# alanqrwang/keymorph

Hardware: AMD Instinct MI355X
Metric: volume-pairs/sec (fwd+bwd) at 256^3, 512 kp, TPS (higher is better)
Workload: dtype f32

## Files before the change

include/keymorph_hip.h:

```cpp
#ifndef KEYMORPH_HIP_H
#define KEYMORPH_HIP_H
#include <stddef.h>
#include <stdint.h>
#ifdef __cplusplus
extern "C" {
#endif

#define KMH_EINVAL (-22)
#define KMH_ABI_VERSION 1
int kmh_abi_version(void);

int kmh_grid_sample3d_fwd(const float* x, const float* grid, float* out, int N, int C, int D, int H,
                          int W, int Do, int Ho, int Wo, int mode, void* stream);
int kmh_grid_sample3d_bwd_grid(const float* x, const float* grid, const float* gout, float* dgrid,
                               int N, int C, int D, int H, int W, int Do, int Ho, int Wo, void* stream);
int kmh_grid_sample3d_bwd_input(const float* grid, const float* gout, float* dx, int N, int C, int D,
                                int H, int W, int Do, int Ho, int Wo, void* stream);

size_t kmh_reduce_ws_bytes(void);
int kmh_mse_fwd(const float* a, const float* b, long long n, float* out, void* ws, void* stream);
int kmh_mse_bwd(const float* a, const float* b, const float* gscale, long long n, float* da, void* stream);
int kmh_warp_mse_fwd(const float* x, const float* grid, const float* fixed, float* out, float* out_loss,
                     int N, int C, int D, int H, int W, int Do, int Ho, int Wo, void* ws, void* stream);
int kmh_warp_mse_fwd_grad(const float* x, const float* grid, const float* fixed, float* out, float* out_loss,
// ... 102 lines not shown
size_t kmh_conv3d_pack_bf_bytes(int Cout, int Cin, int transposed, int terms);
int kmh_conv3d_pack_weight_bf(const float* w, void* packed, int Cout, int Cin, int transposed, int terms,
                              const float* wscale, void* stream);
size_t kmh_conv3d_fwd_bf_stats_ws_bytes(int N, int D, int H, int W, int Cout, int rows_per_wave);
int kmh_conv3d_fwd_bf(const float* x, const float* scale, const float* shift, const float* mask, const void* packed,
                      const float* bias, float* y, int N, int D, int H, int W, int Cin, int Cout, int relu_in,
                      int relu_out, int terms, int rows_per_wave, const float* ascale, const float* wscale,
                      void* stats_ws, double* stats_out, int in_blocked, const float* addend, void* stream);
int kmh_conv3d_fwd_bf_set_dispatch(int mode);
int kmh_conv3d_fwd_bf_split_ok(int N, int D, int H, int W, int Cin, int Cout, int terms);
int kmh_conv3d_fwd_bf_sparse_ok(int N, int D, int H, int W, int Cin, int Cout, int terms);
int kmh_conv3d_fwd_bf_sparse(const float* xp, const unsigned char* winners, const void* packed, const float* bias, float* y,
                             int N, int D, int H, int W, int Cin, int Cout, int relu_out, int terms, const float* ascale,
                             const float* wscale, void* stats_ws, double* stats_out, void* stream);
int kmh_conv3d_fwd_bf_variant(int N, int D, int H, int W, int Cin, int Cout, int terms, int has_mask, int has_addend);
int kmh_conv3d_fwd_bf_pool_ok(int N, int D, int H, int W, int Cin, int Cout, int terms);
int kmh_conv3d_fwd_bf_pool(const float* x, const float* scale, const float* shift, const void* packed, float* yp,
                           unsigned char* arg, int N, int D, int H, int W, int Cin, int Cout, int relu_in, int terms,
                           const float* ascale, const float* wscale, void* stats_ws, double* stats_out, int in_blocked,
                           void* stream);
size_t kmh_conv3d_up2_pack_bytes(int Cout, int Cl, int terms);
int kmh_conv3d_up2_pack_weight(const float* w, void* packed, int Cout, int Ctot, int cofs, int Cl, int terms,
                               const float* wscale, void* stream);
size_t kmh_conv3d_up2_dgrad_pack_bytes(int Cout, int Cl, int terms);
int kmh_conv3d_up2_dgrad_pack_weight(const float* w, void* packed, int Cout, int Ctot, int cofs, int Cl, int terms,
                                     const float* wscale, void* stream);
size_t kmh_conv3d_up2_dgrad_stats_ws_bytes(int N, int Dl, int Hl, int Wl, int Cl);
int kmh_conv3d_up2_dgrad(const float* dz, const void* packed, float* ds, int N, int Dl, int Hl, int Wl, int Cl, int Cout,
                         int terms, const float* dscale, const float* wscale, void* stats_ws, double* stats_out,
                         int in_blocked ,
// ... 158 lines not shown
```

keymorph_amd/_lib.py:

```python
from __future__ import annotations

import ctypes as C
import os

from .build import LIBPATH

_f = C.c_void_p
_i = C.c_int
_ll = C.c_longlong
_sz = C.c_size_t

PROTOS = {
    "kmh_abi_version": (_i, []),
    "kmh_grid_sample3d_fwd": (_i, [_f, _f, _f, _i, _i, _i, _i, _i, _i, _i, _i, _i, _f]),
    "kmh_grid_sample3d_bwd_grid": (_i, [_f, _f, _f, _f, _i, _i, _i, _i, _i, _i, _i, _i, _f]),
    "kmh_grid_sample3d_bwd_input": (_i, [_f, _f, _f, _i, _i, _i, _i, _i, _i, _i, _i, _f]),
    "kmh_reduce_ws_bytes": (_sz, []),
    "kmh_mse_fwd": (_i, [_f, _f, _ll, _f, _f, _f]),
    "kmh_mse_bwd": (_i, [_f, _f, _f, _ll, _f, _f]),
    "kmh_warp_mse_fwd": (_i, [_f, _f, _f, _f, _f, _i, _i, _i, _i, _i, _i, _i, _i, _f, _f]),
    "kmh_warp_mse_fwd_grad": (_i, [_f, _f, _f, _f, _f, _f, _i, _i, _i, _i, _i, _i, _i, _i, _f, _f]),
    "kmh_scale_unless_one": (_i, [_f, _ll, _f, _f]),
    "kmh_dice_sums": (_i, [_f, _f, _i, _ll, _f, _f, _f]),
    "kmh_rows_axpby": (_i, [_f, _f, _f, _f, _i, _ll, _f, _f]),
# ... 40 lines not shown
    "kmh_mi_hist_ranges": (_i, [_f, _f, _f, _i, _ll, _i, _f, _f]),
    "kmh_warp_mi_ws_bytes": (_sz, [_i, _i, _i, _i, _i]),
    "kmh_warp_mi_hist": (_i, [_f, _f, _f, _f, _i, _i, _i, _i, _i, _f, _f]),
    "kmh_warp_mi_bwd": (_i, [_f, _f, _f, _f, _f, _f, _i, _i, _i, _i, _i, _f, _f, _f]),
    "kmh_affine_build_matrix": (_i, [_f, _f, _f, _f, _f, _i, _f]),
    "kmh_affine_points_bwd": (_i, [_f, _f, _f, _f, _f, _i, _i, _f]),
    "kmh_com3d_fwd": (_i, [_f, _f, _f, _i, _i, _i, _i, _i, _f, _f]),
    "kmh_com3d_bwd": (_i, [_f, _f, _f, _f, _i, _i, _i, _i, _i, _f]),
    "kmh_conv3d_pack_weight": (_i, [_f, _f, _i, _i, _i, _f]),
    "kmh_conv3d_fwd": (_i, [_f, _f, _f, _f, _f, _f, _f, _i, _i, _i, _i, _i, _i, _i, _i, _f]),
    "kmh_conv3d_pack_bf_bytes": (_sz, [_i, _i, _i, _i]),
    "kmh_conv3d_pack_weight_bf": (_i, [_f, _f, _i, _i, _i, _i, _f, _f]),
    "kmh_conv3d_fwd_bf": (_i, [_f, _f, _f, _f, _f, _f, _f, _i, _i, _i, _i, _i, _i, _i, _i, _i, _i, _f, _f, _f, _f, _i, _f, _f]),
    "kmh_conv3d_fwd_bf_set_dispatch": (_i, [_i]),
    "kmh_conv3d_fwd_bf_variant": (_i, [_i, _i, _i, _i, _i, _i, _i, _i, _i]),
    "kmh_conv3d_fwd_bf_pool_ok": (_i, [_i, _i, _i, _i, _i, _i, _i]),
    "kmh_conv3d_fwd_bf_split_ok": (_i, [_i, _i, _i, _i, _i, _i, _i]),
    "kmh_conv3d_fwd_bf_sparse_ok": (_i, [_i, _i, _i, _i, _i, _i, _i]),
    "kmh_conv3d_fwd_bf_sparse": (_i, [_f, _f, _f, _f, _f, _i, _i, _i, _i, _i, _i, _i, _i, _f, _f, _f, _f, _f]),
    "kmh_conv3d_fwd_bf_pool": (_i, [_f, _f, _f, _f, _f, _f, _i, _i, _i, _i, _i, _i, _i, _i, _f, _f, _f, _f, _i, _f]),
    "kmh_conv3d_up2_dgrad_pack_bytes": (_sz, [_i, _i, _i]),
    "kmh_conv3d_up2_dgrad_pack_weight": (_i, [_f, _f, _i, _i, _i, _i, _i, _f, _f]),
    "kmh_conv3d_up2_dgrad_stats_ws_bytes": (_sz, [_i, _i, _i, _i, _i]),
    "kmh_conv3d_up2_dgrad": (_i, [_f, _f, _f, _i, _i, _i, _i, _i, _i, _i, _f, _f, _f, _f, _i, _f]),
    "kmh_up2_boxsum": (_i, [_f, _f, _i, _i, _i, _i, _i, _i, _f]),
    "kmh_up2_wgrad_gemm_ws_bytes": (_sz, [_i, _i, _i, _i]),
    "kmh_up2_wgrad_gemm": (_i, [_f, _f, _f, _i, _i, _i, _i, _i, _f, _f, _f, _f, _f, _f]),
    "kmh_up2_wgrad_fold_ok": (_i, [_i, _i, _i]),
    "kmh_up2_wgrad_fold_ws_bytes": (_sz, [_i, _i, _i, _i, _i, _i]),
    "kmh_up2_wgrad_fold": (_i, [_f, _f, _f, _i, _i, _i, _i, _i, _i, _i, _f, _f, _f, _f, _i, _f, _f]),
# ... 178 lines not shown
```

keymorph_amd/csrc/conv_bf.hip:

```cpp
#include <atomic>
#include <cstdio>
#include <cstdlib>
#include "conv_split.h"
#include "stats_final.h"
#include <type_traits>

namespace {

constexpr int TX = 32, TZ = 2;
constexpr int HX = TX + 2, HZ = TZ + 2;
constexpr int NSTEP = 14;
constexpr int BF_TPB = 256;

constexpr int NSTEP_Z = 18;
template <int TERMS>
__global__ __launch_bounds__(256) void pack_weight_bf_kernel(const float* __restrict__ w, __bf16* __restrict__ out,
                                                             int Cout, int Cin, int CoutP, int nchunk,
                                                             int transposed, int zpair,
                                                             const float* __restrict__ wscale ) {
  const int Co = transposed ? Cin : Cout, Ci = transposed ? Cout : Cin;
  const int nstep = zpair ? NSTEP_Z : NSTEP;
  const long long total = (long long)nchunk * nstep * 2 * CoutP * 8;
  for (long long e = (long long)blockIdx.x * 256 + threadIdx.x; e < total; e += (long long)gridDim.x * 256) {
    const int c = (int)(e & 7);
// ... 732 lines not shown
#define KMH_S_DEEP 1
#endif
#ifndef KMH_S_CW
#define KMH_S_CW 1
#endif
#ifndef KMH_S_STAMPALL
#define KMH_S_STAMPALL 0
#endif
#ifndef KMH_S_IL
#define KMH_S_IL 1
#endif
#ifndef KMH_S_DEEP_RING_V
#define KMH_S_DEEP_RING_V 0
#endif

template <int NT, bool ZP = false, bool SPLIT = false, bool POOL = false, bool AMP = false, bool SPARSE = false>
__global__ __launch_bounds__(S_TPB, 1) void conv3_fwd_s_kernel(
    const float* __restrict__ x, const float* __restrict__ scale, const float* __restrict__ shift,
    const bf16x8* __restrict__ wp, const float* __restrict__ bias, float* __restrict__ y, int D, int H, int W, int Cin,
    int Cout, int CoutP, int relu_in, int relu_out, int tiles_x, int tiles_y, int tiles_z, int tiles_zp,
    const float* __restrict__ ascale, const float* __restrict__ wscale, double* __restrict__ stats_partial,
    int in_blocked, const float* __restrict__ addend, int total_items, int N, long long* __restrict__ trace,
    unsigned* __restrict__ pool_arg = nullptr) {
  constexpr int TERMS = 2, MR = ZP ? 4 : S_MR, NST = ZP ? NSTEP_Z : NSTEP;
  static_assert(!ZP || NT == 1, "z-paired tiles are for Cout <= 16");
  static_assert(ZP == SPLIT, "the z-paired tile is launched on pre-split operands only (fp32 operands: conv3_fwd_g_kernel<1, true>)");
  static_assert(!POOL || (NT == 1 && !ZP), "the pooling epilogue is built for the 32-wide tile");
  static_assert(!SPARSE || (SPLIT && ZP && !AMP && TX % 2 == 0 && GTY % 2 == 0 && GTZ % 2 == 0), "pooled operand: the pre-split arm, even brick origins");
  extern __shared__ __attribute__((aligned(16))) unsigned char gsm[];
  int* sOff = reinterpret_cast<int*>(gsm + 2 * S_BUF_BYTES);
  float* sCoef = reinterpret_cast<float*>(gsm + 2 * S_BUF_BYTES + S_OFF_BYTES);
  const int tid = threadIdx.x, lane = tid & 63;
  const int wv = __builtin_amdgcn_readfirstlane(tid >> 6);
  const int li = lane & 31, lh = lane >> 5;
  const int ncog = ZP ? 1 : (Cout + 32 * NT - 1) / (32 * NT);
  const int tyz = (tiles_y + 7) >> 3;
  struct Item { int n, cog, bx, by, bz; };
  const int total_all = N * total_items;
  auto decode = [&](int vb, Item& it) -> bool {
    const int gitem = xcd_remap(vb, total_all);
    it.n = gitem / total_items;
    const int item = gitem - it.n * total_items;
    it.cog = item % ncog;
    const int brick = item / ncog;
    const int lz8 = brick & 7, ly8 = (brick >> 3) & 7, patch = brick >> 6;
    const int pyi = patch % tyz, rest = patch / tyz;
    const int pzi = rest % tiles_zp;
    it.bx = rest / tiles_zp; it.by = pyi * 8 + ly8; it.bz = pzi * 8 + lz8;
// ... 76 lines not shown
      const int v0_ = r * S_TPB + t_, v = v0_ < GPL ? v0_ : GPL - 1;
      const int lx = v % HX, ly = (v / HX) % GHY, lz = v / (HX * GHY);
      int gx = x0 + lx - 1, gy = y0 + ly - 1, gz = z0 + lz - 1;
      const bool in = (v0_ < GPL) && ((unsigned)gx < (unsigned)W) && ((unsigned)gy < (unsigned)H) && ((unsigned)gz < (unsigned)D);
      bits |= (in ? 1u : 0u) << r;
      gx = gx < 0 ? 0 : (gx > W - 1 ? W - 1 : gx);
      gy = gy < 0 ? 0 : (gy > H - 1 ? H - 1 : gy);
      gz = gz < 0 ? 0 : (gz > D - 1 ? D - 1 : gz);
      const int off = ((gz * H + gy) * W + gx) * (in_blocked ? KC : Cin);
      sOff[r * S_TPB + t_] = off;
      sOff[(8 + r) * S_TPB + t_] = off + 4;
    }
    return bits;
  };
  typedef float kmh_f4 __attribute__((ext_vector_type(4)));
  constexpr bool DEEP = (NT == 1) && !ZP && !SPLIT && (KMH_S_DEEP != 0);
  constexpr bool CW = !SPLIT && (KMH_S_CW != 0);
  constexpr int CD = DEEP ? 3 : (CW ? 2 : 1);
  constexpr int RQ = CD + 1;
  kmh_f4 rawq[RQ][2];
  auto raw_issue = [&](int n, int ch, int slot, int off0, int off1) {
    const float* base = sample_base(n) + ch * chunk_stride;
    const float* p0 = base + off0;
    const float* p1 = base + off1;
    if constexpr (CW) {
      asm volatile("global_load_dwordx4 %0, %1, off" : "=v"(rawq[slot][0]) : "v"(p0) : "memory");
      asm volatile("global_load_dwordx4 %0, %1, off" : "=v"(rawq[slot][1]) : "v"(p1) : "memory");
    } else {
      rawq[slot][0] = *reinterpret_cast<const kmh_f4*>(p0);
      rawq[slot][1] = *reinterpret_cast<const kmh_f4*>(p1);
    }
  };
// ... 12 lines not shown
      case 6: asm volatile("s_waitcnt vmcnt(6)" ::: "memory"); break;
      case 7: asm volatile("s_waitcnt vmcnt(7)" ::: "memory"); break;
      case 8: asm volatile("s_waitcnt vmcnt(8)" ::: "memory"); break;
      default: asm volatile("s_waitcnt vmcnt(0)" ::: "memory"); break;
    }
  };
  int coef_n = -1;
  auto fill_coef = [&](int n_) {
    for (int e = tid; e < Cin; e += S_TPB) {
      sCoef[e] = (scale ? scale[n_ * Cin + e] : 1.f) * sA;
      sCoef[S_COEF + e] = (scale ? shift[n_ * Cin + e] : 0.f) * sA;
    }
    coef_n = n_;
  };
  const float relu_floor = relu_in ? 0.f : -__builtin_inff();
  auto convert1 = [&](int ch, unsigned bits, int pb, int i, const kmh_f4 r0, const kmh_f4 r1) {
    const float4 a0 = *reinterpret_cast<const float4*>(sCoef + ch * KC), a1 = *reinterpret_cast<const float4*>(sCoef + ch * KC + 4);
    const float4 b0 = *reinterpret_cast<const float4*>(sCoef + S_COEF + ch * KC), b1 = *reinterpret_cast<const float4*>(sCoef + S_COEF + ch * KC + 4);
    const float csc[8] = {a0.x, a0.y, a0.z, a0.w, a1.x, a1.y, a1.z, a1.w};
    const float csh[8] = {b0.x, b0.y, b0.z, b0.w, b1.x, b1.y, b1.z, b1.w};
    bf16x8* B8 = reinterpret_cast<bf16x8*>(gsm + pb * S_BUF_BYTES);
    const int v = tid + i * S_TPB;
    const float raw[8] = {r0.x, r0.y, r0.z, r0.w, r1.x, r1.y, r1.z, r1.w};
    const bool in = (bits >> i) & 1u;
    const float lo = in ? relu_floor : 0.f, hi = in ? __builtin_inff() : 0.f;
    float val[8];
#pragma unroll
    for (int j = 0; j < 8; ++j) val[j] = __builtin_amdgcn_fmed3f(raw[j] * csc[j] + csh[j], lo, hi);
    bf16x8 parts[TERMS];
    split8<TERMS>(val, parts);
#pragma unroll
    for (int t = 0; t < TERMS; ++t) B8[t * S_PLANE + v] = parts[t];
  };

  auto dma_piece = [&](int n, int ch, int buf, int p, int off) {
    const float* src = sample_base(n) + ch * chunk_stride + off + 4 * (p & 1);
    unsigned char* dst = gsm + buf * S_BUF_BYTES + ((p & 1) * S_PLANE + (p >> 1) * S_TPB + wv * 64) * 16;
    __builtin_amdgcn_global_load_lds((kmh_glb_ptr)src, (kmh_lds_ptr)dst, 16, 0, 0);
  };
  typedef unsigned sp_u4 __attribute__((ext_vector_type(4)));
  const sp_u4* const spTab = reinterpret_cast<const sp_u4*>(sOff);
  kmh_f4 spg[2][2];
  typedef unsigned sp_u2 __attribute__((ext_vector_type(2)));
  sp_u2 spw[2];
  unsigned sph[4], spl[4], spP[4], spM[4], spB = 0;
  auto sp_issue = [&](int n, int ch) {
    const long long cells = vox >> 3;
// ... 115 lines not shown
    for (int t = s_ - BA + 1; t < s_; ++t) yb += NBL + nr(t);
    return yr < yb ? yr : yb;
  };
  auto a_offset = [&](int s) -> int {
    constexpr int last_tap = ZP ? 35 : 26;
    const int tapA = 2 * s, tapB = (2 * s + 1 > last_tap) ? last_tap : 2 * s + 1;
    const int offA = ((tapA / 9) * GHY + (tapA / 3) % 3) * HX + tapA % 3;
    const int offB = ((tapB / 9) * GHY + (tapB / 3) % 3) * HX + tapB % 3;
    return lh ? offB : offA;
  };

  int tr_n = 0;
  auto stamp = [&]() {
    if (trace && blockIdx.x == 0 && tid == 0 && tr_n < 240) trace[tr_n++] = __builtin_readcyclecounter();
  };
  unsigned cv_in = fill_offsets(cur);
  unsigned cv_brick_next = 0u;
  if constexpr (SPARSE) {
    sp_issue(cur.n, 0);
    asm volatile("s_waitcnt vmcnt(0)" ::: "memory");
    sp_tie();
#pragma unroll
    for (int c = 0; c < 2; ++c)
#pragma unroll
      for (int part = 0; part < SP_PARTS; ++part) sp_part(c, part, 0);
  } else if constexpr (SPLIT) {
#pragma unroll
    for (int p = 0; p < S_NLD; ++p) dma_piece(cur.n, 0, 0, p, sOff[(p >> 1) * S_TPB + tid]);
    asm volatile("s_waitcnt vmcnt(0)" ::: "memory");
  } else {
    fill_coef(cur.n);
    __syncthreads();
#pragma unroll
    for (int i = 0; i < S_NCV; ++i) {
      raw_issue(cur.n, 0, 0, sOff[i * S_TPB + tid], sOff[(8 + i) * S_TPB + tid]);
      asm volatile("s_waitcnt vmcnt(0)" ::: "memory");
      if (CW) raw_tie(0);
      convert1(0, cv_in, 0, i, rawq[0][0], rawq[0][1]);
    }
  }
  o0 = lh * CoutP + cur.cog * (32 * NT) + li;
#pragma unroll
  for (int d = 0; d < BA; ++d) b_issue(d);
  if (SPLIT || DEEP) asm volatile("s_waitcnt vmcnt(0)" ::: "memory");
  int pb = 0;
  for (;;) {
    const bool more = next_item(vb, nxt);
    const int co0 = cur.cog * (32 * NT);
    const int n = cur.n;
    const int boff = lh * CoutP + co0 + li;
    f32x16 acc[MR][NT];
#pragma unroll
    for (int m = 0; m < MR; ++m)
#pragma unroll
      for (int t = 0; t < NT; ++t)
#pragma unroll
        for (int r = 0; r < 16; ++r) acc[m][t][r] = 0.f;

    for (int ch = 0; ch < nchunk; ++ch) {
      stamp();
      asm volatile("s_waitcnt lgkmcnt(0)" ::: "memory");
      __builtin_amdgcn_s_barrier();
      stamp();
      const bf16x8* sIn = reinterpret_cast<const bf16x8*>(gsm + pb * S_BUF_BYTES);
      const bool last_ch = ch + 1 == nchunk;
      const int nn = (last_ch && more) ? nxt.n : n, nch = last_ch ? 0 : ch + 1;
      unsigned cv_next = last_ch ? 0u : cv_in;
      if (!SPLIT && nn != coef_n) {
        fill_coef(nn);
        __syncthreads();
      }
      const int co0n = ((last_ch && more) ? nxt.cog : cur.cog) * (32 * NT);
      int vr = vrow;
      asm volatile("" : "+v"(vr));
      int dof0 = 0, dof1 = 0;
      bf16x8 a[2][MR][TERMS];
      {
        const int ab = vr + a_offset(0);
#pragma unroll
        for (int m = 0; m < MR; ++m)
// ... 61 lines not shown
        } else {
        if (SPLIT || !(s >= 1 + CD && s < 9 + CD)) __builtin_amdgcn_sched_group_barrier(0x100, 64, 0);
        if (!SPLIT && s >= 1 + CD && s < 9 + CD) {
          __builtin_amdgcn_sched_group_barrier(0x100, 64, 0);
          __builtin_amdgcn_sched_group_barrier(0x008, 6, 0);
#pragma unroll
          for (int k = 0; k < NMF - 6; ++k) {
            __builtin_amdgcn_sched_group_barrier(0x002, 3, 0);
            __builtin_amdgcn_sched_group_barrier(0x008, 1, 0);
          }
        }
        }
        __builtin_amdgcn_sched_barrier(0);
        __builtin_amdgcn_sched_barrier(0);
        if (KMH_S_STAMPALL || s == 0 || s == 9 || s == NST - 1) stamp();
      }
      if (!last_ch) pb ^= 1;
    }

    if (SPLIT || DEEP) asm volatile("s_waitcnt vmcnt(0)" ::: "memory");
    const int x0 = cur.bx * TX, y0 = cur.by * GTY, z0 = cur.bz * GTZ;
    constexpr int CH = 32 * NT;
    constexpr int L4 = CH / 4;
    constexpr int VPI = 64 / L4;
    const long long sbrick = ((long long)n * tiles_z * tiles_y * tiles_x + ((long long)cur.bz * tiles_y + cur.by) * tiles_x + cur.bx);
    unsigned char* sEp = gsm + pb * S_BUF_BYTES;
    float* tile0 = reinterpret_cast<float*>(sEp) + wv * (2 * 32 * CH);
    const int c4 = lane % L4, vx = lane / L4;
    const int col = 4 * c4;
    const int pl = ZP ? col >> 4 : 0;
// ... 109 lines not shown
#pragma unroll
      for (int j = 0; j < 4; ++j) {
        d1[j] = (double)st1[j]; d2[j] = (double)st2[j];
#pragma unroll
        for (int o = L4; o < 64; o <<= 1) { d1[j] += __shfl_xor(d1[j], o); d2[j] += __shfl_xor(d2[j], o); }
      }
      if (POOL) stamp();
      __syncthreads();
      double* sred = reinterpret_cast<double*>(sEp);
      if (lane < L4) {
#pragma unroll
        for (int j = 0; j < 4; ++j) { sred[((wv * CH) + col + j) * 2] = d1[j]; sred[((wv * CH) + col + j) * 2 + 1] = d2[j]; }
      }
      __syncthreads();
      const int ncol = ZP ? 16 : CH;
      if (tid < 2 * ncol) {
        const int k = tid & 1, c = tid >> 1;
        const int cch = ZP ? c : co0 + c;
        if (cch < Cout) {
          double sum = 0.0;
#pragma unroll
          for (int w4 = 0; w4 < 4; ++w4) {
            sum += sred[(w4 * CH + c) * 2 + k];
            if (ZP) sum += sred[(w4 * CH + 16 + c) * 2 + k];
          }
          stats_partial[(sbrick * Cout + cch) * 2 + k] = sum;
        }
      }
    }
    stamp();
    if (!more) break;
    cur = nxt;
    cv_in = cv_brick_next;
    pb ^= 1;
  }
  asm volatile("s_waitcnt vmcnt(0)" ::: "memory");
}

}
static inline bool use_zpair(int Cout) { return Cout <= 16; }

KMH_API size_t kmh_conv3d_pack_bf_bytes(int Cout, int Cin, int transposed, int terms) {
  const int Co = transposed ? Cin : Cout, Ci = transposed ? Cout : Cin;
  return (size_t)((Ci + 7) / 8) * terms * (use_zpair(Co) ? NSTEP_Z : NSTEP) * 2 * cout_pad(Co) * 8 * sizeof(__bf16);
}

KMH_API int kmh_conv3d_pack_weight_bf(const float* w, void* packed, int Cout, int Cin, int transposed, int terms,
                                      const float* wscale, void* stream) {
  const int Co = transposed ? Cin : Cout, Ci = transposed ? Cout : Cin;
  const int nchunk = (Ci + 7) / 8, CoutP = cout_pad(Co), zp = use_zpair(Co);
  const long long total = (long long)nchunk * (zp ? NSTEP_Z : NSTEP) * 2 * CoutP * 8;
// ... 63 lines not shown
  if (int e = allow_lds(conv3_fwd_g_kernel<NT, ZP, POOL>, G_LDS_BYTES)) return e;
  const PersistentGrid g = persistent_grid(N, D, H, W, ZP ? 1 : ceil_div(Cout, 32 * NT));
  long long* trace = trace_begin(s);
  conv3_fwd_g_kernel<NT, ZP, POOL><<<dim3(g.wgs), G_TPB, G_LDS_BYTES, s>>>(x, scale, shift, wp, bias, y, D, H, W, Cin, Cout, CoutP,
                                                                           relu_in, relu_out, g.tx, g.ty, g.tz, g.tzp, ascale, wscale,
                                                                           stats_out ? stats_ws : nullptr, in_blocked, addend,
                                                                           g.total, N, trace, pool_arg);
  trace_end(trace, s, "KMH_G_TRACE NT=%d ZP=%d Cin=%d Cout=%d D=%d:", NT, (int)ZP, Cin, Cout, D);
  return finish_stats(stats_ws, g.tx * g.ty * g.tz, Cout, N, stats_out, s);
}

template <int NT, bool ZP = false, bool SPLIT = false, bool POOL = false>
static int launch_fwd_s(bool amp, const float* x, const float* scale, const float* shift, const bf16x8* wp, const float* bias, float* y,
                        int N, int D, int H, int W, int Cin, int Cout, int CoutP, int relu_in, int relu_out,
                        const float* ascale, const float* wscale, double* stats_ws, double* stats_out, hipStream_t s,
                        int in_blocked, const float* addend, unsigned* pool_arg = nullptr) {
  if (int e = allow_lds(conv3_fwd_s_kernel<NT, ZP, SPLIT, POOL>, S_LDS_BYTES)) return e;
  const PersistentGrid g = persistent_grid(N, D, H, W, ZP ? 1 : ceil_div(Cout, 32 * NT));
  long long* trace = trace_begin(s);
#define KMH_S_ARGS x, scale, shift, wp, bias, y, D, H, W, Cin, Cout, CoutP, relu_in, relu_out, g.tx, g.ty, g.tz, g.tzp, ascale, wscale, \
                   stats_out ? stats_ws : nullptr, in_blocked, addend, g.total, N, trace, pool_arg
  if (amp) {
    if (int e = allow_lds(conv3_fwd_s_kernel<NT, ZP, SPLIT, POOL, true>, S_LDS_BYTES)) return e;
    conv3_fwd_s_kernel<NT, ZP, SPLIT, POOL, true><<<dim3(g.wgs), S_TPB, S_LDS_BYTES, s>>>(KMH_S_ARGS);
  } else
    conv3_fwd_s_kernel<NT, ZP, SPLIT, POOL><<<dim3(g.wgs), S_TPB, S_LDS_BYTES, s>>>(KMH_S_ARGS);
#undef KMH_S_ARGS
  trace_end(trace, s, "KMH_G_TRACE fwd_s NT=%d ZP=%d SPLIT=%d POOL=%d Cin=%d Cout=%d D=%d:", NT, (int)ZP, (int)SPLIT, (int)POOL, Cin, Cout, D);
  return finish_stats(stats_ws, g.tx * g.ty * g.tz, Cout, N, stats_out, s);
}

static std::atomic<int> g_fwd_g_mode{-1};
static int fwd_g_mode() {
  int m = g_fwd_g_mode.load(std::memory_order_relaxed);
  if (m < 0) {
    m = getenv("KEYMORPH_FWD_G") ? atoi(getenv("KEYMORPH_FWD_G")) : 1;
    if (m < 0 || m > 2) m = 1;
    g_fwd_g_mode.store(m, std::memory_order_relaxed);
  }
  return m;
}

static bool fwd_s_on() {
  static const bool on = !(getenv("KEYMORPH_FWD_S") && atoi(getenv("KEYMORPH_FWD_S")) == 0);
  return on;
}

static bool fwd_g_ok(bool mask, bool addend, int N, int D, int H, int W, int Cin, int Cout, int terms) {
  const int mode = fwd_g_mode();
  if (!mode || terms != 2 || mask || (Cin & 7) || (Cout & 3)) return false;
  if (use_zpair(Cout) && addend) return false;
  if ((long long)D * H * W * (Cin > Cout ? Cin : Cout) >= (1ll << 31)) return false;
  const long long wgs = (long long)N * ceil_div(W, TX) * ceil_div(H, GTY) * ceil_div(D, GTZ) *
                        (use_zpair(Cout) ? 1 : ceil_div(Cout, 64));
  return wgs >= (mode == 2 ? 1 : 512);
}

KMH_API int kmh_conv3d_fwd_bf_set_dispatch(int mode) {
  if (mode < 0 || mode > 2) return -22;
  const int old = fwd_g_mode();
  g_fwd_g_mode.store(mode, std::memory_order_relaxed);
  return old;
}

KMH_API int kmh_conv3d_fwd_bf_variant(int N, int D, int H, int W, int Cin, int Cout, int terms, int has_mask,
                                      int has_addend) {
  if (!fwd_g_ok(has_mask != 0, has_addend != 0, N, D, H, W, Cin, Cout, terms)) return 0;
  return use_zpair(Cout) ? 3 : (Cout > 32 ? 2 : 1);
}

KMH_API int kmh_conv3d_fwd_bf_split_ok(int N, int D, int H, int W, int Cin, int Cout, int terms) {
  if (!use_zpair(Cout) || Cin > S_COEF) return 0;
  if (((long long)D * H * W + 1) * KC >= (1ll << 31)) return 0;
  if (N <= 0 || terms != 2 || (Cin & 7) || (Cout & 3)) return 0;
  if ((long long)D * H * W * (Cin > Cout ? Cin : Cout) >= (1ll << 31)) return 0;
  return 1;
}

KMH_API int kmh_conv3d_fwd_bf_sparse_ok(int N, int D, int H, int W, int Cin, int Cout, int terms) {
  if (terms != 2 || ((D | H | W) & 1) || D < 2 || H < 2 || W < 2) return 0;
  return kmh_conv3d_fwd_bf_split_ok(N, D, H, W, Cin, Cout, terms);
}

// ... 16 lines not shown

KMH_API int kmh_conv3d_fwd_bf_pool_ok(int N, int D, int H, int W, int Cin, int Cout, int terms) {
  return (Cout > 16 && Cout <= 32 && D >= 2 && H >= 2 && W >= 2 && fwd_g_ok(false, false, N, D, H, W, Cin, Cout, terms)) ? 1 : 0;
}

KMH_API int kmh_conv3d_fwd_bf_pool(const float* x, const float* scale, const float* shift, const void* packed, float* yp,
                                   unsigned char* arg, int N, int D, int H, int W, int Cin, int Cout, int relu_in,
                                   int terms, const float* ascale, const float* wscale, void* stats_ws, double* stats_out,
                                   int in_blocked, void* stream) {
  const bool amp = kmh_take_amp(terms);
  if (!kmh_conv3d_fwd_bf_pool_ok(N, D, H, W, Cin, Cout, terms) || !ascale || !wscale || !yp || !arg) return -22;
  if (((uintptr_t)yp & 15) || ((uintptr_t)arg & 3)) return -22;
  if (fwd_s_on() && Cin <= S_COEF)
    return launch_fwd_s<1, false, false, true>(amp, x, scale, shift, (const bf16x8*)packed, nullptr, yp, N, D, H, W, Cin, Cout,
                                               cout_pad(Cout), relu_in, 1, ascale, wscale, (double*)stats_ws, stats_out,
                                               (hipStream_t)stream, in_blocked, nullptr, (unsigned*)arg);
  return launch_fwd_g<1, false, true>(x, scale, shift, (const bf16x8*)packed, nullptr, yp, N, D, H, W, Cin, Cout,
                                      cout_pad(Cout), relu_in, 1, ascale, wscale, (double*)stats_ws, stats_out,
                                      (hipStream_t)stream, in_blocked, nullptr, (unsigned*)arg);
}

static inline int fwd_bf_rows(int Cout) {
  return use_zpair(Cout) ? 8 : 4;
}

KMH_API size_t kmh_conv3d_fwd_bf_stats_ws_bytes(int N, int D, int H, int W, int Cout, int rows_per_wave) {
  return (size_t)N * ceil_div(W, TX) * ceil_div(H, fwd_bf_rows(Cout)) * ceil_div(D, TZ) * Cout * 2 *
         sizeof(double);
}

KMH_API int kmh_conv3d_fwd_bf(const float* x, const float* scale, const float* shift, const float* mask,
// ... 11 lines not shown
  if (terms != 2 && terms != 3) return -22;
  if (addend && use_zpair(Cout)) return -22;
  if (in_blocked && ((Cin & 7) || mask)) return -22;
  if (in_blocked == 2) {
    if (!kmh_conv3d_fwd_bf_split_ok(N, D, H, W, Cin, Cout, terms) || scale || shift || relu_in || addend || !ascale || !wscale)
      return -22;
    return launch_fwd_s<1, true, true>(amp, x, nullptr, nullptr, wp, bias, y, N, D, H, W, Cin, Cout, CoutP, 0, relu_out, ascale, wscale,
                                       (double*)stats_ws, stats_out, s, 2, nullptr);
  }
  if (terms == 2 && (!ascale || !wscale)) return -22;
  const bool deep = terms == 2 && Cout <= 32 && D >= 16 && (long long)D * H * W >= (1ll << 21);
  if (fwd_g_ok(mask != nullptr, addend != nullptr, N, D, H, W, Cin, Cout, terms)) {
    if (use_zpair(Cout)) return launch_fwd_g<1, true>(x, scale, shift, wp, bias, y, N, D, H, W, Cin, Cout, CoutP, relu_in, relu_out, ascale, wscale, (double*)stats_ws, stats_out, s, in_blocked, addend);
    if (fwd_s_on() && Cin <= S_COEF) {
      if (Cout > 32) return launch_fwd_s<2>(amp, x, scale, shift, wp, bias, y, N, D, H, W, Cin, Cout, CoutP, relu_in, relu_out, ascale, wscale, (double*)stats_ws, stats_out, s, in_blocked, addend);
      return launch_fwd_s<1>(amp, x, scale, shift, wp, bias, y, N, D, H, W, Cin, Cout, CoutP, relu_in, relu_out, ascale, wscale, (double*)stats_ws, stats_out, s, in_blocked, addend);
    }
    if (Cout > 32) return launch_fwd_g<2, false>(x, scale, shift, wp, bias, y, N, D, H, W, Cin, Cout, CoutP, relu_in, relu_out, ascale, wscale, (double*)stats_ws, stats_out, s, in_blocked, addend);
    return launch_fwd_g<1, false>(x, scale, shift, wp, bias, y, N, D, H, W, Cin, Cout, CoutP, relu_in, relu_out, ascale, wscale, (double*)stats_ws, stats_out, s, in_blocked, addend);
  }
  if (use_zpair(Cout)) {
    if (terms == 2 && deep) return launch_fwd_bf<1, 2, 2, true, 2>(x, scale, shift, mask, wp, bias, y, N, D, H, W, Cin, Cout, CoutP, relu_in, relu_out, ascale, wscale, (double*)stats_ws, stats_out, s, in_blocked);
    if (terms == 2) return launch_fwd_bf<1, 2, 2, true>(x, scale, shift, mask, wp, bias, y, N, D, H, W, Cin, Cout, CoutP, relu_in, relu_out, ascale, wscale, (double*)stats_ws, stats_out, s, in_blocked);
    return launch_fwd_bf<1, 3, 2, true>(x, scale, shift, mask, wp, bias, y, N, D, H, W, Cin, Cout, CoutP, relu_in, relu_out, ascale, wscale, (double*)stats_ws, stats_out, s, in_blocked);
  }
  const long long wgs4 = (long long)N * ceil_div(W, TX) * ceil_div(H, 8) * ceil_div(D, 2) * ceil_div(Cout, 64);
  const bool small_grid = wgs4 < 2048;
  if (small_grid && terms == 2 && Cout % 128 == 0) KMH_BF_CALL(4, 2, 2);
  if (terms == 2 && Cout > 64 && Cout <= 96) KMH_BF_CALL(3, 2, 2);
  if (Cout > 32) {
    if (terms == 2) { if (mr == 4 && !small_grid) KMH_BF_CALL(2, 2, 4); else KMH_BF_CALL(2, 2, 2); }
// ... 8 lines not shown
```

Before: 15.75.

## Add warp-specialized producer/consumer variant of persistent conv3d forward kernel

Adds a warp-specialized version of the persistent 32-wide conv3d forward kernel that launches twice the threads per workgroup. One half loads fp32 activations, applies scale/shift, splits them to bf16 terms and stores them to LDS, while the other half only runs the MFMA loop with register-prefetched weights. The intent is to overlap global loads and conversion with matrix math instead of interleaving them in the same waves. It is enabled by default for the plain and pooled non-AMP paths. The cost is doubled thread count, barrier lockstep between the roles, and added register and scheduling complexity.

```diff
diff --git a/include/keymorph_hip.h b/include/keymorph_hip.h
--- a/include/keymorph_hip.h
+++ b/include/keymorph_hip.h
@@ -140,6 +140,7 @@
                              int N, int D, int H, int W, int Cin, int Cout, int relu_out, int terms, const float* ascale,
                              const float* wscale, void* stats_ws, double* stats_out, void* stream);
 int kmh_conv3d_fwd_bf_variant(int N, int D, int H, int W, int Cin, int Cout, int terms, int has_mask, int has_addend);
+int kmh_conv3d_fwd_bf_ws(int N, int D, int H, int W, int Cin, int Cout, int terms, int has_mask, int has_addend, int pool);
 int kmh_conv3d_fwd_bf_pool_ok(int N, int D, int H, int W, int Cin, int Cout, int terms);
 int kmh_conv3d_fwd_bf_pool(const float* x, const float* scale, const float* shift, const void* packed, float* yp,
                            unsigned char* arg, int N, int D, int H, int W, int Cin, int Cout, int relu_in, int terms,
diff --git a/keymorph_amd/_lib.py b/keymorph_amd/_lib.py
--- a/keymorph_amd/_lib.py
+++ b/keymorph_amd/_lib.py
@@ -78,6 +78,7 @@
     "kmh_conv3d_fwd_bf": (_i, [_f, _f, _f, _f, _f, _f, _f, _i, _i, _i, _i, _i, _i, _i, _i, _i, _i, _f, _f, _f, _f, _i, _f, _f]),
     "kmh_conv3d_fwd_bf_set_dispatch": (_i, [_i]),
     "kmh_conv3d_fwd_bf_variant": (_i, [_i, _i, _i, _i, _i, _i, _i, _i, _i]),
+    "kmh_conv3d_fwd_bf_ws": (_i, [_i, _i, _i, _i, _i, _i, _i, _i, _i, _i]),
     "kmh_conv3d_fwd_bf_pool_ok": (_i, [_i, _i, _i, _i, _i, _i, _i]),
     "kmh_conv3d_fwd_bf_split_ok": (_i, [_i, _i, _i, _i, _i, _i, _i]),
     "kmh_conv3d_fwd_bf_sparse_ok": (_i, [_i, _i, _i, _i, _i, _i, _i]),
diff --git a/keymorph_amd/csrc/conv_bf.hip b/keymorph_amd/csrc/conv_bf.hip
--- a/keymorph_amd/csrc/conv_bf.hip
+++ b/keymorph_amd/csrc/conv_bf.hip
@@ -770,24 +770,26 @@
 #define KMH_S_DEEP_RING_V 0
 #endif
 
-template <int NT, bool ZP = false, bool SPLIT = false, bool POOL = false, bool AMP = false, bool SPARSE = false>
-__global__ __launch_bounds__(S_TPB, 1) void conv3_fwd_s_kernel(
+template <int NT, bool ZP, bool SPLIT, bool POOL, bool AMP, bool SPARSE, bool WS>
+__device__ __forceinline__ void conv3_fwd_s_body(
     const float* __restrict__ x, const float* __restrict__ scale, const float* __restrict__ shift,
     const bf16x8* __restrict__ wp, const float* __restrict__ bias, float* __restrict__ y, int D, int H, int W, int Cin,
     int Cout, int CoutP, int relu_in, int relu_out, int tiles_x, int tiles_y, int tiles_z, int tiles_zp,
     const float* __restrict__ ascale, const float* __restrict__ wscale, double* __restrict__ stats_partial,
     int in_blocked, const float* __restrict__ addend, int total_items, int N, long long* __restrict__ trace,
-    unsigned* __restrict__ pool_arg = nullptr) {
+    unsigned* __restrict__ pool_arg) {
   constexpr int TERMS = 2, MR = ZP ? 4 : S_MR, NST = ZP ? NSTEP_Z : NSTEP;
   static_assert(!ZP || NT == 1, "z-paired tiles are for Cout <= 16");
   static_assert(ZP == SPLIT, "the z-paired tile is launched on pre-split operands only (fp32 operands: conv3_fwd_g_kernel<1, true>)");
   static_assert(!POOL || (NT == 1 && !ZP), "the pooling epilogue is built for the 32-wide tile");
   static_assert(!SPARSE || (SPLIT && ZP && !AMP && TX % 2 == 0 && GTY % 2 == 0 && GTZ % 2 == 0), "pooled operand: the pre-split arm, even brick origins");
+  static_assert(!WS || (NT == 1 && !ZP && !SPLIT && !AMP), "wave roles: the 32-wide tile on an fp32 operand");
   extern __shared__ __attribute__((aligned(16))) unsigned char gsm[];
   int* sOff = reinterpret_cast<int*>(gsm + 2 * S_BUF_BYTES);
   float* sCoef = reinterpret_cast<float*>(gsm + 2 * S_BUF_BYTES + S_OFF_BYTES);
-  const int tid = threadIdx.x, lane = tid & 63;
+  const int tid = WS ? (int)(threadIdx.x & (S_TPB - 1)) : (int)threadIdx.x, lane = tid & 63;
   const int wv = __builtin_amdgcn_readfirstlane(tid >> 6);
+  const int role = WS ? __builtin_amdgcn_readfirstlane((int)threadIdx.x / S_TPB) : 0;
   const int li = lane & 31, lh = lane >> 5;
   const int ncog = ZP ? 1 : (Cout + 32 * NT - 1) / (32 * NT);
   const int tyz = (tiles_y + 7) >> 3;
@@ -894,8 +896,8 @@
     return bits;
   };
   typedef float kmh_f4 __attribute__((ext_vector_type(4)));
-  constexpr bool DEEP = (NT == 1) && !ZP && !SPLIT && (KMH_S_DEEP != 0);
-  constexpr bool CW = !SPLIT && (KMH_S_CW != 0);
+  constexpr bool DEEP = (NT == 1) && !ZP && !SPLIT && !WS && (KMH_S_DEEP != 0);
+  constexpr bool CW = !SPLIT && !WS && (KMH_S_CW != 0);
   constexpr int CD = DEEP ? 3 : (CW ? 2 : 1);
   constexpr int RQ = CD + 1;
   kmh_f4 rawq[RQ][2];
@@ -938,11 +940,7 @@
     coef_n = n_;
   };
   const float relu_floor = relu_in ? 0.f : -__builtin_inff();
-  auto convert1 = [&](int ch, unsigned bits, int pb, int i, const kmh_f4 r0, const kmh_f4 r1) {
-    const float4 a0 = *reinterpret_cast<const float4*>(sCoef + ch * KC), a1 = *reinterpret_cast<const float4*>(sCoef + ch * KC + 4);
-    const float4 b0 = *reinterpret_cast<const float4*>(sCoef + S_COEF + ch * KC), b1 = *reinterpret_cast<const float4*>(sCoef + S_COEF + ch * KC + 4);
-    const float csc[8] = {a0.x, a0.y, a0.z, a0.w, a1.x, a1.y, a1.z, a1.w};
-    const float csh[8] = {b0.x, b0.y, b0.z, b0.w, b1.x, b1.y, b1.z, b1.w};
+  auto convert_store = [&](const float (&csc)[8], const float (&csh)[8], unsigned bits, int pb, int i, const kmh_f4 r0, const kmh_f4 r1) {
     bf16x8* B8 = reinterpret_cast<bf16x8*>(gsm + pb * S_BUF_BYTES);
     const int v = tid + i * S_TPB;
     const float raw[8] = {r0.x, r0.y, r0.z, r0.w, r1.x, r1.y, r1.z, r1.w};
@@ -955,6 +953,31 @@
     split8<TERMS>(val, parts);
 #pragma unroll
     for (int t = 0; t < TERMS; ++t) B8[t * S_PLANE + v] = parts[t];
+  };
+  auto convert1 = [&](int ch, unsigned bits, int pb, int i, const kmh_f4 r0, const kmh_f4 r1) {
+    const float4 a0 = *reinterpret_cast<const float4*>(sCoef + ch * KC), a1 = *reinterpret_cast<const float4*>(sCoef + ch * KC + 4);
+    const float4 b0 = *reinterpret_cast<const float4*>(sCoef + S_COEF + ch * KC), b1 = *reinterpret_cast<const float4*>(sCoef + S_COEF + ch * KC + 4);
+    const float csc[8] = {a0.x, a0.y, a0.z, a0.w, a1.x, a1.y, a1.z, a1.w};
+    const float csh[8] = {b0.x, b0.y, b0.z, b0.w, b1.x, b1.y, b1.z, b1.w};
+    convert_store(csc, csh, bits, pb, i, r0, r1);
+  };
+  auto produce_stage = [&](int n_, int ch, unsigned bits, int buf) {
+    float csc[8], csh[8];
+#pragma unroll
+    for (int j = 0; j < 8; ++j) {
+      csc[j] = (scale ? scale[n_ * Cin + ch * KC + j] : 1.f) * sA;
+      csh[j] = (scale ? shift[n_ * Cin + ch * KC + j] : 0.f) * sA;
+      asm volatile("" : "+v"(csc[j]), "+v"(csh[j]));
+    }
+    const float* base = sample_base(n_) + ch * chunk_stride;
+    kmh_f4 r[S_NCV][2];
+#pragma unroll
+    for (int i = 0; i < S_NCV; ++i) {
+      r[i][0] = *reinterpret_cast<const kmh_f4*>(base + sOff[i * S_TPB + tid]);
+      r[i][1] = *reinterpret_cast<const kmh_f4*>(base + sOff[(8 + i) * S_TPB + tid]);
+    }
+#pragma unroll
+    for (int i = 0; i < S_NCV; ++i) convert_store(csc, csh, bits, buf, i, r[i][0], r[i][1]);
   };
 
   auto dma_piece = [&](int n, int ch, int buf, int p, int off) {
@@ -1100,9 +1123,55 @@
   auto stamp = [&]() {
     if (trace && blockIdx.x == 0 && tid == 0 && tr_n < 240) trace[tr_n++] = __builtin_readcyclecounter();
   };
-  unsigned cv_in = fill_offsets(cur);
+  auto stage_barrier = [&]() {
+    asm volatile("s_waitcnt lgkmcnt(0)" ::: "memory");
+    __builtin_amdgcn_s_barrier();
+  };
+  if constexpr (WS) {
+    if (role) {
+      unsigned bits = fill_offsets(cur), bits_next = 0u;
+      produce_stage(cur.n, 0, bits, 0);
+      int buf = 0;
+      for (;;) {
+        const bool more = next_item(vb, nxt);
+        for (int ch = 0; ch < nchunk; ++ch) {
+          stage_barrier();
+          if (ch + 1 < nchunk) {
+            produce_stage(cur.n, ch + 1, bits, buf ^ 1);
+            buf ^= 1;
+          } else if (more) {
+            bits_next = fill_offsets(nxt);
+            produce_stage(nxt.n, 0, bits_next, buf ^ 1);
+          }
+        }
+        stage_barrier();
+        if (stats_partial) { stage_barrier(); stage_barrier(); }
+        if (!more) return;
+        cur = nxt;
+        bits = bits_next;
+        buf ^= 1;
+      }
+    }
+  }
+  unsigned cv_in = WS ? 0u : fill_offsets(cur);
   unsigned cv_brick_next = 0u;
-  if constexpr (SPARSE) {
+  constexpr int WS_BD = 2;
+  static_assert((NST - WS_BD) % WS_BD == 0, "the refills run through the steps in order, a stage's first ones in slots 0 ..");
+  bf16x8 wbq[WS_BD][TERMS];
+  const bf16x8* const wp1 = wp + term_stride;
+  int wo = 0;
+  auto ws_b_stage = [&](int ch_, int co0_) { wo = ch_ * TERMS * (int)term_stride + lh * CoutP + co0_ + li; };
+  auto ws_b_load = [&](int slot) {
+    asm volatile("" : "+v"(wo));
+    wbq[slot][0] = wp[wo];
+    wbq[slot][1] = wp1[wo];
+    wo += (int)step_stride;
+  };
+  if constexpr (WS) {
+    ws_b_stage(0, cur.cog * 32);
+#pragma unroll
+    for (int d = 0; d < WS_BD; ++d) ws_b_load(d);
+  } else if constexpr (SPARSE) {
     sp_issue(cur.n, 0);
     asm volatile("s_waitcnt vmcnt(0)" ::: "memory");
     sp_tie();
@@ -1126,8 +1195,10 @@
     }
   }
   o0 = lh * CoutP + cur.cog * (32 * NT) + li;
-#pragma unroll
-  for (int d = 0; d < BA; ++d) b_issue(d);
+  if constexpr (!WS) {
+#pragma unroll
+    for (int d = 0; d < BA; ++d) b_issue(d);
+  }
   if (SPLIT || DEEP) asm volatile("s_waitcnt vmcnt(0)" ::: "memory");
   int pb = 0;
   for (;;) {
@@ -1145,11 +1216,54 @@
 
     for (int ch = 0; ch < nchunk; ++ch) {
       stamp();
-      asm volatile("s_waitcnt lgkmcnt(0)" ::: "memory");
-      __builtin_amdgcn_s_barrier();
+      stage_barrier();
       stamp();
       const bf16x8* sIn = reinterpret_cast<const bf16x8*>(gsm + pb * S_BUF_BYTES);
       const bool last_ch = ch + 1 == nchunk;
+      if constexpr (WS) {
+        const int nch = last_ch ? 0 : ch + 1;
+        const int co0n = ((last_ch && more) ? nxt.cog : cur.cog) * 32;
+        int vr = vrow;
+        asm volatile("" : "+v"(vr));
+        bf16x8 a[2][4][TERMS];
+        int lhv = lh;
+        asm volatile("" : "+v"(lhv));
+        auto a_read = [&](int hs) {
+          const int tapA = 2 * (hs >> 1), tapB = tapA + 1 > 26 ? 26 : tapA + 1;
+          const int offA = ((tapA / 9) * GHY + (tapA / 3) % 3) * HX + tapA % 3;
+          const int offB = ((tapB / 9) * GHY + (tapB / 3) % 3) * HX + tapB % 3;
+          const int ab = vr + offA + lhv * (offB - offA);
+#pragma unroll
+          for (int m = 0; m < 4; ++m)
+#pragma unroll
+            for (int q = 0; q < TERMS; ++q) a[hs & 1][m][q] = sIn[q * S_PLANE + ab + arow(4 * (hs & 1) + m)];
+        };
+        a_read(0);
+#pragma unroll
+        for (int hs = 0; hs < 2 * NST; ++hs) {
+          const int s = hs >> 1, h = 4 * (hs & 1);
+          if (hs + 1 < 2 * NST) a_read(hs + 1);
+#pragma unroll
+          for (int q3 = 0; q3 < 3; ++q3)
+#pragma unroll
+            for (int m = 0; m < 4; ++m)
+              acc[h + m][0] = mfma16<TERMS>(a[hs & 1][m][q3 == 0 ? 1 : 0], wbq[s % WS_BD][q3 == 1 ? 1 : 0], acc[h + m][0]);
+          if (hs & 1) {
+            if (s + WS_BD == NST) ws_b_stage(nch, co0n);
+            ws_b_load(s % WS_BD);
+          }
+#pragma unroll
+          for (int k = 0; k < 12; ++k) {
+            __builtin_amdgcn_sched_group_barrier(0x008, 1, 0);
+            if (k < 8 && hs + 1 < 2 * NST) __builtin_amdgcn_sched_group_barrier(0x100, 1, 0);
+          }
+          __builtin_amdgcn_sched_barrier(0);
+        }
+        if (last_ch) {
+#pragma unroll
+          for (int d = 0; d < WS_BD; ++d) { asm volatile("" : "+v"(wbq[d][0])); asm volatile("" : "+v"(wbq[d][1])); }
+        }
+      } else {
       const int nn = (last_ch && more) ? nxt.n : n, nch = last_ch ? 0 : ch + 1;
       unsigned cv_next = last_ch ? 0u : cv_in;
       if (!SPLIT && nn != coef_n) {
@@ -1241,6 +1355,7 @@
         __builtin_amdgcn_sched_barrier(0);
         __builtin_amdgcn_sched_barrier(0);
         if (KMH_S_STAMPALL || s == 0 || s == 9 || s == NST - 1) stamp();
+      }
       }
       if (!last_ch) pb ^= 1;
     }
@@ -1380,8 +1495,10 @@
       }
       __syncthreads();
       const int ncol = ZP ? 16 : CH;
-      if (tid < 2 * ncol) {
-        const int k = tid & 1, c = tid >> 1;
+      int ts = tid;
+      if constexpr (WS) asm volatile("" : "+v"(ts));
+      if (ts < 2 * ncol) {
+        const int k = ts & 1, c = ts >> 1;
         const int cch = ZP ? c : co0 + c;
         if (cch < Cout) {
           double sum = 0.0;
@@ -1401,6 +1518,32 @@
     pb ^= 1;
   }
   asm volatile("s_waitcnt vmcnt(0)" ::: "memory");
+}
+
+template <int NT, bool ZP = false, bool SPLIT = false, bool POOL = false, bool AMP = false, bool SPARSE = false>
+__global__ __launch_bounds__(S_TPB, 1) void conv3_fwd_s_kernel(
+    const float* __restrict__ x, const float* __restrict__ scale, const float* __restrict__ shift,
+    const bf16x8* __restrict__ wp, const float* __restrict__ bias, float* __restrict__ y, int D, int H, int W, int Cin,
+    int Cout, int CoutP, int relu_in, int relu_out, int tiles_x, int tiles_y, int tiles_z, int tiles_zp,
+    const float* __restrict__ ascale, const float* __restrict__ wscale, double* __restrict__ stats_partial,
+    int in_blocked, const float* __restrict__ addend, int total_items, int N, long long* __restrict__ trace,
+    unsigned* __restrict__ pool_arg = nullptr) {
+  conv3_fwd_s_body<NT, ZP, SPLIT, POOL, AMP, SPARSE, false>(
+      x, scale, shift, wp, bias, y, D, H, W, Cin, Cout, CoutP, relu_in, relu_out, tiles_x, tiles_y, tiles_z, tiles_zp, ascale, wscale,
+      stats_partial, in_blocked, addend, total_items, N, trace, pool_arg);
+}
+
+template <bool POOL>
+__global__ __launch_bounds__(2 * S_TPB, 1) void conv3_fwd_ws_kernel(
+    const float* __restrict__ x, const float* __restrict__ scale, const float* __restrict__ shift,
+    const bf16x8* __restrict__ wp, const float* __restrict__ bias, float* __restrict__ y, int D, int H, int W, int Cin,
+    int Cout, int CoutP, int relu_in, int relu_out, int tiles_x, int tiles_y, int tiles_z, int tiles_zp,
+    const float* __restrict__ ascale, const float* __restrict__ wscale, double* __restrict__ stats_partial,
+    int in_blocked, const float* __restrict__ addend, int total_items, int N, long long* __restrict__ trace,
+    unsigned* __restrict__ pool_arg = nullptr) {
+  conv3_fwd_s_body<1, false, false, POOL, false, false, true>(
+      x, scale, shift, wp, bias, y, D, H, W, Cin, Cout, CoutP, relu_in, relu_out, tiles_x, tiles_y, tiles_z, tiles_zp, ascale, wscale,
+      stats_partial, in_blocked, addend, total_items, N, trace, pool_arg);
 }
 
 }
@@ -1494,7 +1637,7 @@
 static int launch_fwd_s(bool amp, const float* x, const float* scale, const float* shift, const bf16x8* wp, const float* bias, float* y,
                         int N, int D, int H, int W, int Cin, int Cout, int CoutP, int relu_in, int relu_out,
                         const float* ascale, const float* wscale, double* stats_ws, double* stats_out, hipStream_t s,
-                        int in_blocked, const float* addend, unsigned* pool_arg = nullptr) {
+                        int in_blocked, const float* addend, unsigned* pool_arg = nullptr, bool ws = false) {
   if (int e = allow_lds(conv3_fwd_s_kernel<NT, ZP, SPLIT, POOL>, S_LDS_BYTES)) return e;
   const PersistentGrid g = persistent_grid(N, D, H, W, ZP ? 1 : ceil_div(Cout, 32 * NT));
   long long* trace = trace_begin(s);
@@ -1503,6 +1646,12 @@
   if (amp) {
     if (int e = allow_lds(conv3_fwd_s_kernel<NT, ZP, SPLIT, POOL, true>, S_LDS_BYTES)) return e;
     conv3_fwd_s_kernel<NT, ZP, SPLIT, POOL, true><<<dim3(g.wgs), S_TPB, S_LDS_BYTES, s>>>(KMH_S_ARGS);
+  } else if (ws) {
+    if constexpr (NT == 1 && !ZP && !SPLIT) {
+      if (int e = allow_lds(conv3_fwd_ws_kernel<POOL>, S_LDS_BYTES)) return e;
+      conv3_fwd_ws_kernel<POOL><<<dim3(g.wgs), 2 * S_TPB, S_LDS_BYTES, s>>>(KMH_S_ARGS);
+    } else
+      return -22;
   } else
     conv3_fwd_s_kernel<NT, ZP, SPLIT, POOL><<<dim3(g.wgs), S_TPB, S_LDS_BYTES, s>>>(KMH_S_ARGS);
 #undef KMH_S_ARGS
@@ -1526,6 +1675,13 @@
   return on;
 }
 
+constexpr bool kWsPlainDefault = true, kWsPoolDefault = true;
+static bool fwd_ws_take(bool pool, bool amp) {
+  static const int mode = getenv("KEYMORPH_FWD_WS") ? (atoi(getenv("KEYMORPH_FWD_WS")) != 0 ? 1 : 0) : -1;
+  if (amp) return false;
+  return mode < 0 ? (pool ? kWsPoolDefault : kWsPlainDefault) : mode == 1;
+}
+
 static bool fwd_g_ok(bool mask, bool addend, int N, int D, int H, int W, int Cin, int Cout, int terms) {
   const int mode = fwd_g_mode();
   if (!mode || terms != 2 || mask || (Cin & 7) || (Cout & 3)) return false;
@@ -1547,6 +1703,13 @@
                                       int has_addend) {
   if (!fwd_g_ok(has_mask != 0, has_addend != 0, N, D, H, W, Cin, Cout, terms)) return 0;
   return use_zpair(Cout) ? 3 : (Cout > 32 ? 2 : 1);
+}
+
+KMH_API int kmh_conv3d_fwd_bf_ws(int N, int D, int H, int W, int Cin, int Cout, int terms, int has_mask, int has_addend, int pool) {
+  if (!fwd_g_ok(has_mask != 0, has_addend != 0, N, D, H, W, Cin, Cout, terms == 1 ? 2 : terms)) return 0;
+  if (use_zpair(Cout) || Cout > 32 || !fwd_s_on() || Cin > S_COEF) return 0;
+  if (pool && (has_mask || has_addend || D < 2 || H < 2 || W < 2)) return 0;
+  return fwd_ws_take(pool != 0, terms == 1) ? 1 : 0;
 }
 
 KMH_API int kmh_conv3d_fwd_bf_split_ok(int N, int D, int H, int W, int Cin, int Cout, int terms) {
@@ -1593,7 +1756,7 @@
   if (fwd_s_on() && Cin <= S_COEF)
     return launch_fwd_s<1, false, false, true>(amp, x, scale, shift, (const bf16x8*)packed, nullptr, yp, N, D, H, W, Cin, Cout,
                                                cout_pad(Cout), relu_in, 1, ascale, wscale, (double*)stats_ws, stats_out,
-                                               (hipStream_t)stream, in_blocked, nullptr, (unsigned*)arg);
+                                               (hipStream_t)stream, in_blocked, nullptr, (unsigned*)arg, fwd_ws_take(true, amp));
   return launch_fwd_g<1, false, true>(x, scale, shift, (const bf16x8*)packed, nullptr, yp, N, D, H, W, Cin, Cout,
                                       cout_pad(Cout), relu_in, 1, ascale, wscale, (double*)stats_ws, stats_out,
                                       (hipStream_t)stream, in_blocked, nullptr, (unsigned*)arg);
@@ -1635,7 +1798,8 @@
     if (use_zpair(Cout)) return launch_fwd_g<1, true>(x, scale, shift, wp, bias, y, N, D, H, W, Cin, Cout, CoutP, relu_in, relu_out, ascale, wscale, (double*)stats_ws, stats_out, s, in_blocked, addend);
     if (fwd_s_on() && Cin <= S_COEF) {
       if (Cout > 32) return launch_fwd_s<2>(amp, x, scale, shift, wp, bias, y, N, D, H, W, Cin, Cout, CoutP, relu_in, relu_out, ascale, wscale, (double*)stats_ws, stats_out, s, in_blocked, addend);
-      return launch_fwd_s<1>(amp, x, scale, shift, wp, bias, y, N, D, H, W, Cin, Cout, CoutP, relu_in, relu_out, ascale, wscale, (double*)stats_ws, stats_out, s, in_blocked, addend);
+      return launch_fwd_s<1>(amp, x, scale, shift, wp, bias, y, N, D, H, W, Cin, Cout, CoutP, relu_in, relu_out, ascale, wscale, (double*)stats_ws, stats_out, s, in_blocked, addend,
+                             nullptr, fwd_ws_take(false, amp));
     }
     if (Cout > 32) return launch_fwd_g<2, false>(x, scale, shift, wp, bias, y, N, D, H, W, Cin, Cout, CoutP, relu_in, relu_out, ascale, wscale, (double*)stats_ws, stats_out, s, in_blocked, addend);
     return launch_fwd_g<1, false>(x, scale, shift, wp, bias, y, N, D, H, W, Cin, Cout, CoutP, relu_in, relu_out, ascale, wscale, (double*)stats_ws, stats_out, s, in_blocked, addend);
```

Result: no change. 15.79 (median of 6 runs) (+0.3%).
